# GEOS-ESM/QuickChem

Hardware: AMD Instinct MI355X
Metric: OH gridcells/sec (XGBoost predict), C360 L72 batch (higher is better)
Workload: dtype f32

## Files before the change

quickchem_amd/csrc/kernels.hip:

```cpp
#include <hip/hip_runtime.h>

#include <atomic>

#include <cstdint>

#include "kernels.hpp"

namespace ohx {

namespace {

constexpr int kWave = 64;
constexpr int kBlock = 256;
constexpr int kWavesPerBlock = kBlock / kWave;

typedef float f4u __attribute__((ext_vector_type(4), aligned(4)));
typedef unsigned int u32x2 __attribute__((ext_vector_type(2)));
typedef unsigned int u32x4 __attribute__((ext_vector_type(4)));
typedef const __attribute__((address_space(3))) char* lds_cptr;
typedef const __attribute__((address_space(3))) u32x4* lds_u32x4_ptr;
typedef __attribute__((address_space(3))) uint32_t* lds_u32_ptr;
typedef __attribute__((address_space(3))) void* lds_void_ptr;

__device__ __forceinline__ __amdgpu_buffer_rsrc_t make_rsrc(const void* p, uint32_t bytes) {
// ... 126 lines not shown
        x[g] = ((a.is2d_mask >> f) & 1u) ? src[at2] : __builtin_nontemporal_load(src + at3);
      }
    }
#pragma unroll
    for (uint32_t g = 0; g < GROUP; ++g) {
      const uint32_t f = f0 + g;
      float v = x[g];
      if (f == a.pl_feature) {
        asm volatile("");
        v = v / 100.0f;
      }
      any_inf |= f < nfeat && is_inf(v);
      if (!missing_is_nan && v == a.missing) v = qnan;
      if (!valid) v = 0.0f;
      lane_nan |= f < nfeat && (v != v);
      if (f < nfeat) tile[f * kWave] = v;
    }
  }
  if (any_inf && !is_inf(a.missing) && a.flags) atomicOr(a.flags, kFlagInfInput);
  return lane_nan;
}

struct CellAt {
  uint64_t at3, at2;
};
__device__ __forceinline__ CellAt cell_at(const FieldsArgs& a, uint64_t plane, uint64_t m) {
  const uint64_t k = m / plane, col = m - k * plane;
  return CellAt{a.level_stride ? k * a.level_stride + col : m, col};
}
__device__ __forceinline__ uint64_t level_floats(const FieldsArgs& a, uint64_t plane) {
  return a.level_stride ? a.level_stride : plane;
}

__device__ __forceinline__ float pow10_f32(float x) {
  double y = (double)x * 3.321928094887362;
  y = y < -1100.0 ? -1100.0 : (y > 1100.0 ? 1100.0 : y);
  const double n = __builtin_rint(y);
  const double f = y - n;
  double p = 4.44553827187081e-10;
  p = __builtin_fma(p, f, 7.054911620801121e-09);
  p = __builtin_fma(p, f, 1.0178086009239696e-07);
  p = __builtin_fma(p, f, 1.3215486790144305e-06);
  p = __builtin_fma(p, f, 1.5252733804059838e-05);
  p = __builtin_fma(p, f, 0.00015403530393381606);
  p = __builtin_fma(p, f, 0.0013333558146428441);
  p = __builtin_fma(p, f, 0.009618129107628477);
  p = __builtin_fma(p, f, 0.055504108664821576);
  p = __builtin_fma(p, f, 0.2402265069591007);
  p = __builtin_fma(p, f, 0.6931471805599453);
  p = __builtin_fma(p, f, 1.0);
  return (float)__builtin_ldexp(p, (int)n);
}

__device__ __forceinline__ void store_oh(const FieldsArgs& a, float* __restrict__ out, float* __restrict__ margin_out,
                                         uint64_t slab_out, uint64_t m, uint64_t at3, float acc) {
  if (margin_out) margin_out[m] = acc;
  float oh = acc;
  if (a.apply_pow10) oh = pow10_f32(acc);
  oh = oh * a.scale;
  out[slab_out + at3] = oh;
}

struct Row27 {
  f4u v[7];
};

__device__ __forceinline__ void load_row27(Row27& r, const float* __restrict__ rows, uint64_t row) {
  const float* p = rows + row * 27u;
#pragma unroll
  for (int q = 0; q < 6; ++q) r.v[q] = __builtin_nontemporal_load(reinterpret_cast<const f4u*>(p + 4 * q));
#pragma unroll
  for (int q = 0; q < 3; ++q) r.v[6][q] = __builtin_nontemporal_load(p + 24 + q);
}

__device__ __forceinline__ bool store_row27(float* __restrict__ tile, const Row27& r, bool valid, float missing,
                                            bool missing_is_nan, uint32_t* flags) {
  bool any_nan = false, any_inf = false;
  const float qnan = __builtin_nanf("");
#pragma unroll
  for (int f = 0; f < 27; ++f) {
    float x = r.v[f / 4][f % 4];
    if (!valid) x = 0.0f;
    any_inf |= is_inf(x);
    if (!missing_is_nan && x == missing) x = qnan;
    any_nan |= (x != x);
    tile[f * kWave] = x;
  }
  if (any_inf && !is_inf(missing) && flags) atomicOr(flags, kFlagInfInput);
  return any_nan;
}

// ... 25 lines not shown
  }
}

__device__ __forceinline__ bool store_pieces(float* __restrict__ tile_base, const Row27& r, const PredictArgs& a,
                                             uint64_t vmask, int lane, bool missing_is_nan) {
  bool any_nan = false, any_inf = false;
  const float qnan = __builtin_nanf("");
  asm volatile("" : "+v"(lane));
  const uint32_t ppr = 27u << (a.run_log - 2u);
  const bool all_valid = vmask == ~0ull;
#pragma unroll
  for (int q = 0; q < 7; ++q) {
    const uint32_t p = (uint32_t)lane + 64u * (uint32_t)q;
    if (p < kPiecesPerTile) {
      const uint32_t g = div27(p) >> (a.run_log - 2u);
      const uint32_t w4 = 4u * (p - g * ppr);
      const uint32_t col0 = run_first_lane(g, a.run_log, a.run_lo_bits);
      uint32_t rr = div27(w4);
      uint32_t f = w4 - 27u * rr;
#pragma unroll
      for (int c = 0; c < 4; ++c) {
        const uint32_t col = col0 | (rr << a.run_lo_bits);
        float x = r.v[q][c];
        if (!all_valid && !((vmask >> col) & 1ull)) x = 0.0f;
        any_inf |= is_inf(x);
        if (!missing_is_nan && x == a.missing) x = qnan;
        any_nan |= (x != x);
        tile_base[f * kWave + col] = x;
        ++f;
        if (f == 27u) {
          f = 0u;
          ++rr;
        }
      }
    }
  }
  if (any_inf && !is_inf(a.missing) && a.flags) atomicOr(a.flags, kFlagInfInput);
  return any_nan;
}


template <int CHAINS, bool HAS_MISSING>
__device__ __forceinline__ float walk_packed(__amdgpu_buffer_rsrc_t nodes, const uint32_t* __restrict__ roots,
                                             uint32_t t0, uint32_t t1, float acc, const float* __restrict__ tile) {
  for (uint32_t t = t0; t < t1; t += CHAINS) {
    uint2 nd[CHAINS];
    uint32_t cur[CHAINS];
#pragma unroll
    for (int c = 0; c < CHAINS; ++c) {
      const uint32_t tt = (t + c < t1) ? t + c : t1 - 1;
      cur[c] = roots[tt];
      nd[c] = load_node8(nodes, cur[c]);
    }
    bool more;
    do {
      float x[CHAINS];
#pragma unroll
      for (int c = 0; c < CHAINS; ++c) x[c] = tile[(nd[c].y & 31u) * kWave];
      more = false;
#pragma unroll
      for (int c = 0; c < CHAINS; ++c) {
        const uint32_t m = nd[c].y;
        bool go_left = x[c] < __uint_as_float(nd[c].x);
        if (HAS_MISSING) go_left = go_left || ((x[c] != x[c]) && (m & 32u));
        const uint32_t n = (m >> 6) - (go_left ? 1u : 0u);
        cur[c] = (m != 0u) ? n : cur[c];
// ... 24 lines not shown
  }
  return acc;
}


__device__ __forceinline__ bool go_left_or_default(float x, float thr, bool default_left) {
  const bool lt = x < thr;
  const bool missing = x != x;
  return lt | (missing & default_left);
}

using lane_mask = uint64_t;
constexpr int kFcmpOrdered = 7, kFcmpNotLess = 11 , kIcmpEq = 32;

__device__ __forceinline__ uint32_t pick(lane_mask m, uint32_t if_clear, uint32_t if_set) {
  uint32_t r;
  asm("v_cndmask_b32_e64 %0, %1, %2, %3" : "=v"(r) : "v"(if_clear), "v"(if_set), "s"(m));
  return r;
}

__device__ __forceinline__ lane_mask right_or_default(float x, float thr, uint32_t w, uint32_t default_left_bit) {
  const lane_mask not_less = __builtin_amdgcn_fcmpf(x, thr, kFcmpNotLess);
  const lane_mask number = __builtin_amdgcn_fcmpf(x, x, kFcmpOrdered);
  const lane_mask default_right = __builtin_amdgcn_uicmp(w & default_left_bit, 0u, kIcmpEq);
  return not_less & (number | default_right);
}

__device__ __forceinline__ uint32_t double_and_carry(uint32_t v, lane_mask carry) {
  uint32_t r;
  asm("v_addc_co_u32_e64 %0, vcc, %1, %1, %2" : "=v"(r) : "v"(v), "s"(carry) : "vcc");
  return r;
}

template <int CHAINS, bool HAS_MISSING, bool LAST>
__device__ __forceinline__ void super_step(u32x4 (&s)[CHAINS], uint32_t (&rel)[CHAINS], uint32_t (&leafb)[CHAINS],
                                           const char* __restrict__ tile_b) {
  float x0[CHAINS], x1[CHAINS];
  uint32_t thr1[CHAINS], f1[CHAINS];
  bool l0[CHAINS];
  lane_mask r0[CHAINS];
#pragma unroll
  for (int c = 0; c < CHAINS; ++c) {
    asm volatile("" : "+v"(s[c]));
    x0[c] = *reinterpret_cast<const float*>(tile_b + (s[c].w & 0x1F00u));
  }
#pragma unroll
  for (int c = 0; c < CHAINS; ++c) {
    const uint32_t w = s[c].w;
    if constexpr (HAS_MISSING) {
      r0[c] = right_or_default(x0[c], __uint_as_float(s[c].x), w, 32u);
      thr1[c] = pick(r0[c], s[c].y, s[c].z);
      f1[c] = (w >> pick(r0[c], 0u, 13u)) & 31u;
    } else {
      const bool l = x0[c] < __uint_as_float(s[c].x);
      l0[c] = l;
      thr1[c] = l ? s[c].y : s[c].z;
      f1[c] = (w >> (l ? 0u : 13u)) & 31u;
    }
    if (!LAST) x1[c] = *reinterpret_cast<const float*>(tile_b + (f1[c] << 8));
  }
#pragma unroll
  for (int c = 0; c < CHAINS; ++c) {
    const uint32_t w = s[c].w;
    leafb[c] = (f1[c] == 31u) ? thr1[c] : leafb[c];
    if (!LAST) {
      const uint32_t g = w >> 18;
      if constexpr (HAS_MISSING) {
        const lane_mask r1 = right_or_default(x1[c], __uint_as_float(thr1[c]), w, pick(r0[c], 64u, 128u));
        rel[c] = double_and_carry(double_and_carry(g, r0[c]), r1);
      } else {
        const bool l1 = x1[c] < __uint_as_float(thr1[c]);
        const lane_mask right0 = __builtin_amdgcn_ballot_w64(!l0[c]), right1 = __builtin_amdgcn_ballot_w64(!l1);
        rel[c] = double_and_carry(double_and_carry(g, right0), right1);
      }
    }
  }
}

template <int CHAINS, bool HAS_MISSING, class Fetch>
__device__ __forceinline__ void super_step_by_chain(u32x4 (&s)[CHAINS], uint32_t (&rel)[CHAINS], uint32_t (&leafb)[CHAINS],
                                                    const char* __restrict__ tile_b, Fetch fetch) {
  asm volatile("" : "+v"(s[0]));
  float x0_next = *reinterpret_cast<const float*>(tile_b + (s[0].w & 0x1F00u));
#pragma unroll
  for (int c = 0; c < CHAINS; ++c) {
    const uint32_t w = s[c].w;
    const float x0 = x0_next;
    if (c + 1 < CHAINS) {
      asm volatile("" : "+v"(s[c + 1]));
      x0_next = *reinterpret_cast<const float*>(tile_b + (s[c + 1].w & 0x1F00u));
    }
    uint32_t thr1, f1;
    bool l0 = false;
    lane_mask r0 = 0;
    if constexpr (HAS_MISSING) {
      r0 = right_or_default(x0, __uint_as_float(s[c].x), w, 32u);
      thr1 = pick(r0, s[c].y, s[c].z);
      f1 = (w >> pick(r0, 0u, 13u)) & 31u;
    } else {
      l0 = x0 < __uint_as_float(s[c].x);
      thr1 = l0 ? s[c].y : s[c].z;
      f1 = (w >> (l0 ? 0u : 13u)) & 31u;
    }
    const float x1 = *reinterpret_cast<const float*>(tile_b + (f1 << 8));
    const uint32_t g = w >> 18;
    if constexpr (HAS_MISSING) {
      const lane_mask r1 = right_or_default(x1, __uint_as_float(thr1), w, pick(r0, 64u, 128u));
      rel[c] = double_and_carry(double_and_carry(g, r0), r1);
    } else {
      const bool l1 = x1 < __uint_as_float(thr1);
      const lane_mask right0 = __builtin_amdgcn_ballot_w64(!l0), right1 = __builtin_amdgcn_ballot_w64(!l1);
      rel[c] = double_and_carry(double_and_carry(g, right0), right1);
    }
    s[c] = fetch(c, rel[c]);
    leafb[c] = (f1 == 31u) ? thr1 : leafb[c];
    __builtin_amdgcn_sched_barrier(0);
  }
}

constexpr uint32_t kFirstTrees = kFirstStepTrees;
constexpr uint32_t kFirstBytes = kFirstTrees * 2 * 16;

template <int CHAINS>
__device__ __forceinline__ void take_from_lanes(u32x4 (&s)[CHAINS], const u32x4 (&top)[CHAINS],
                                                const uint32_t (&rel)[CHAINS]) {
#pragma unroll
  for (int c = 0; c < CHAINS; ++c) {
    const int a = (int)(rel[c] << 2);
    s[c].x = (uint32_t)__builtin_amdgcn_ds_bpermute(a, (int)top[c].x);
    s[c].y = (uint32_t)__builtin_amdgcn_ds_bpermute(a, (int)top[c].y);
    s[c].z = (uint32_t)__builtin_amdgcn_ds_bpermute(a, (int)top[c].z);
    s[c].w = (uint32_t)__builtin_amdgcn_ds_bpermute(a, (int)top[c].w);
  }
}

template <int CHAINS, bool HAS_MISSING, bool TOPS>
__device__ __forceinline__ float walk_super(const uint4* __restrict__ nodes, const SuperTreeHead* __restrict__ heads,
                                            uint32_t t0, uint32_t t1, float acc, const float* __restrict__ tile,
                                            const char* __restrict__ first, uint32_t nfirst, uint32_t nodes_bytes,
                                            float* __restrict__ leaf_out = nullptr) {
  if (t0 >= t1) return acc;
  const __amdgpu_buffer_rsrc_t forest = make_rsrc(nodes, nodes_bytes);
  const uint32_t lane_id = threadIdx.x & (kWave - 1);
  const uint32_t top_off = (lane_id < kSuperTopSlots ? lane_id : kSuperTopSlots - 1u) << 4;
  const lds_cptr first_lds = (lds_cptr)first;
  const u32x4* __restrict__ nodes_v = reinterpret_cast<const u32x4*>(nodes);
  const char* tile_b = reinterpret_cast<const char*>(tile);
  SuperTreeHead hn[CHAINS];
// ... 329 lines not shown
  const uint64_t addr = reinterpret_cast<uint64_t>(fr.super);
  rg.desc.x = (uint32_t)__builtin_amdgcn_readfirstlane((int)(uint32_t)addr);
  rg.desc.y = (uint32_t)__builtin_amdgcn_readfirstlane((int)((uint32_t)(addr >> 32) & 0xFFFFu));
  rg.desc.z = (uint32_t)__builtin_amdgcn_readfirstlane((int)fr.super_bytes);
  rg.desc.w = 0x00020000u;
  rg.forest = make_rsrc(fr.super, fr.super_bytes);
  rg.heads = heads;
  rg.t0 = t0;
  rg.t1 = t1;
  rg.ngroups = (t1 - t0 + kRingChains - 1) / kRingChains;
  rg.total = rounds * rg.ngroups;
  rg.g = 0;
  rg.gave_up = false;
  if (threadIdx.x < kWave) {
    ring_stage(rg, t0, 0u, lane);
    asm volatile("s_waitcnt vmcnt(0)" ::: "memory");
  }
  if (threadIdx.x < (uint32_t)kRingWaves) ring_store(rg.progress + threadIdx.x, 0u);
  if (threadIdx.x == 0) {
    ring_store(rg.filled, 1u);
    ring_store(rg.claim, 1u);
    ring_store(rg.abort, 0u);
  }
  __syncthreads();
}

template <bool HAS_MISSING>
__device__ __forceinline__ float ring_walk_group(const SuperTreeHead (&h)[kRingChains], uint32_t ntrees_here,
                                                 __amdgpu_buffer_rsrc_t forest, const float* __restrict__ tile,
                                                 lds_cptr tops, float acc, lds_u32_ptr publish_to,
                                                 uint32_t publish_value, bool ahead) {
  constexpr int CHAINS = kRingChains;
  const char* tile_b = reinterpret_cast<const char*>(tile);
  __builtin_amdgcn_s_setprio(1);
  u32x4 s[CHAINS];
  uint32_t rel[CHAINS], leafb[CHAINS];
  float xr[CHAINS];
#pragma unroll
  for (int c = 0; c < CHAINS; ++c) xr[c] = tile[(h[c].root_meta & 31u) * kWave];
#pragma unroll
  for (int c = 0; c < CHAINS; ++c) {
    bool l = xr[c] < h[c].root_thr;
    if (HAS_MISSING) l = go_left_or_default(xr[c], h[c].root_thr, (h[c].root_meta & 32u) != 0u);
    rel[c] = 4u + (((h[c].root_meta & 0x100u) && !l) ? 1u : 0u);
    leafb[c] = 0u;
  }
  uint32_t nsteps = h[0].steps;
#pragma unroll
  for (int c = 1; c < CHAINS; ++c) nsteps = h[c].steps > nsteps ? h[c].steps : nsteps;
  nsteps = nsteps < kRingSteps ? kRingSteps : nsteps;
#pragma unroll
  for (int c = 0; c < CHAINS; ++c) s[c] = *(lds_u32x4_ptr)(tops + (uint32_t)c * kRingTreeBytes + (rel[c] << 4));
#pragma unroll
  for (uint32_t step = 1; step < kRingSteps; ++step) {
    if (step == 2 && !ahead) __builtin_amdgcn_s_setprio(2);
    super_step<CHAINS, HAS_MISSING, false>(s, rel, leafb, tile_b);
#pragma unroll
    for (int c = 0; c < CHAINS; ++c) s[c] = *(lds_u32x4_ptr)(tops + (uint32_t)c * kRingTreeBytes + (rel[c] << 4));
  }
  if (publish_to != nullptr) {
    asm volatile("s_waitcnt vmcnt(0)" ::: "memory");
    if ((threadIdx.x & (kWave - 1)) == 0) ring_store(publish_to, publish_value);
  }
  if (ahead) __builtin_amdgcn_s_setprio(2);
  else __builtin_amdgcn_s_setprio(3);
  uint32_t base[CHAINS];
#pragma unroll
  for (int c = 0; c < CHAINS; ++c) base[c] = h[c].base;
  for (uint32_t step = kRingSteps; step < nsteps; ++step)
    super_step_by_chain<CHAINS, HAS_MISSING>(s, rel, leafb, tile_b, [&](int c, uint32_t record) -> u32x4 {
      return __builtin_amdgcn_raw_buffer_load_b128(forest, (int)((base[c] + record) << 4), 0, 0);
    });
  super_step<CHAINS, HAS_MISSING, true>(s, rel, leafb, tile_b);
  __builtin_amdgcn_s_setprio(1);
#pragma unroll
  for (int c = 0; c < CHAINS; ++c)
    if ((uint32_t)c < ntrees_here) acc += __uint_as_float(leafb[c]);
  return acc;
}

__device__ __forceinline__ bool ring_aborted(const TopRing& rg) {
  return __builtin_amdgcn_readfirstlane((int)ring_load(rg.abort)) != 0;
}

__device__ __forceinline__ void ring_give_up(TopRing& rg, int lane) {
  rg.gave_up = true;
  if (lane == 0) ring_store(rg.abort, 1u);
}

__device__ __forceinline__ float ring_walk_tile(TopRing& rg, float acc, const float* __restrict__ tile, bool live,
                                                bool wave_nan, int lane, int wave) {
  if (rg.gave_up) return acc;
  for (uint32_t p = 0; p < rg.ngroups; ++p, ++rg.g) {
    const uint32_t g = rg.g;
    const uint32_t t = rg.t0 + p * kRingChains;
    uint32_t won = 0;
    uint32_t filled_now = 0;
    if (lane == 0) {
      uint32_t expected = g + 1u;
      const bool may = g + 1u < rg.total && !rg.gave_up;
      filled_now = ring_load(rg.filled);
      if (may) won = __hip_atomic_compare_exchange_strong(rg.claim, &expected, g + 2u, __ATOMIC_RELAXED, __ATOMIC_RELAXED,
                                                          __HIP_MEMORY_SCOPE_WORKGROUP) ? 1u : 0u;
    }
    won = (uint32_t)__builtin_amdgcn_readfirstlane((int)won);
    filled_now = (uint32_t)__builtin_amdgcn_readfirstlane((int)filled_now);
// ... 107 lines not shown
        keep = this_valid && !mine;
        wave_nan = false;
      }
    }
    const float acc = ring_walk_tile(rg, fr.base_score, tile, live, wave_nan, lane, wave);
    if (live && keep && !rg.gave_up) __builtin_nontemporal_store(acc, out + this_row);
    tile_id = next;
  }
  if (rg.gave_up && a.flags && lane == 0) atomicExch(a.flags + 2, a.train_id);
}

__global__ __launch_bounds__(kRingBlock) __attribute__((amdgpu_waves_per_eu(4))) void predict_fields_ring_kernel(
    DeviceForest fr, FieldsArgs a, const SuperTreeHead* __restrict__ heads, float* __restrict__ out,
    float* __restrict__ margin_out) {
  extern __shared__ float lds[];
  const int lane = threadIdx.x & (kWave - 1);
  const int wave = threadIdx.x / kWave;
  float* tile = lds + (size_t)wave * 27 * kWave + lane;
  const bool missing_is_nan = a.missing != a.missing;
  const uint64_t plane = (uint64_t)a.im * (uint64_t)a.jm;
  const uint64_t nrow = plane * (uint64_t)(a.k2 - a.k1 + 1);
  const uint64_t slab = level_floats(a, plane) * (uint64_t)(a.k1 - a.src_k0);
  const uint64_t slab_out = level_floats(a, plane) * (uint64_t)(a.k1 - a.out_k0);
  uint32_t block = blockIdx.x;
  if (a.xcd_remap && (gridDim.x & 7u) == 0u) block = (blockIdx.x & 7u) * (gridDim.x >> 3) + (blockIdx.x >> 3);
  const uint64_t wave_id = (uint64_t)block * kRingWaves + wave;
  const uint64_t nwaves = (uint64_t)gridDim.x * kRingWaves;
  const uint64_t first_tile = a.tile_begin + (uint64_t)block * kRingWaves;
  if (first_tile >= a.tile_end) return;
  const uint32_t rounds = (uint32_t)((a.tile_end - first_tile + nwaves - 1) / nwaves);
  TopRing rg;
  ring_begin(rg, reinterpret_cast<char*>(lds + (size_t)kRingWaves * 27 * kWave), fr, heads, a.tree_begin, a.tree_end, rounds);
  uint64_t tile_id = a.tile_begin + wave_id;
  for (uint32_t r = 0; r < rounds; ++r, tile_id += nwaves) {
    bool valid = false;
    uint64_t m = 0;
    if (tile_id < a.tile_end) m = tile_row(a.shape, tile_id, lane, nrow, &valid);
    const bool live = __any(valid);
    const CellAt at = cell_at(a, plane, valid ? m : 0);
    const bool lane_nan = live && fill_tile_fields(a, tile, 27u, at.at3, at.at2, slab, valid, missing_is_nan);
    bool wave_nan = __any(lane_nan);
    bool keep = valid;
    if (wave_nan && a.defer_count != nullptr && a.defer_cap == 0u) {
      if ((tile_id & 7u) == 0u) {
        const uint32_t n = 8u * (uint32_t)__popcll(__ballot(lane_nan && valid));
        if (lane == 0) atomicAdd(a.defer_count, n);
      }
    } else if (wave_nan && a.defer_count != nullptr) {
      const bool leaves = lane_nan && valid;
      const uint64_t who = __ballot(leaves);
      const uint32_t n = (uint32_t)__popcll(who);
      uint32_t at = 0;
      if (lane == 0) at = atomicAdd(a.defer_count, n);
      at = (uint32_t)__builtin_amdgcn_readfirstlane((int)at);
      if (at + n <= a.defer_cap) {
        if (leaves) a.defer_list[at + (uint32_t)__popcll(who & ((1ull << lane) - 1ull))] = (uint32_t)m;
        keep = valid && !lane_nan;
        wave_nan = false;
      }
    }
    const float acc = ring_walk_tile(rg, fr.base_score, tile, live, wave_nan, lane, wave);
    if (keep && !rg.gave_up) store_oh(a, out, margin_out, slab_out, m, at.at3, acc);
  }
  if (rg.gave_up && a.flags && lane == 0) atomicExch(a.flags + 2, a.train_id);
}

__global__ __launch_bounds__(kBlock) void combine_leaves_kernel(PredictArgs a, float base_score, float* __restrict__ out) {
  const int lane = threadIdx.x & (kWave - 1);
  const uint64_t ntiles = a.tile_end - a.tile_begin, nwaves = (uint64_t)gridDim.x * kWavesPerBlock;
  const uint32_t ntree = a.tree_end - a.tree_begin;
  for (uint64_t w = (uint64_t)blockIdx.x * kWavesPerBlock + threadIdx.x / kWave; w < ntiles; w += nwaves) {
    bool valid;
    const uint64_t row = launch_row(a, a.tile_begin + w, lane, &valid);
    if (!__any(valid)) continue;
    const float* leaves = a.leaf_buf + (size_t)w * ntree * kWave + lane;
    float acc = base_score;
#pragma unroll 4
    for (uint32_t t = 0; t < ntree; ++t) acc += leaves[(size_t)t * kWave];
    if (valid) out[row] = acc;
  }
}

template <bool PRED_LEAF>
__global__ __launch_bounds__(kBlock) void predict_rows_direct_kernel(DeviceForest fr, PredictArgs a) {
  const uint4* nodes = reinterpret_cast<const uint4*>(fr.wide);
  const bool missing_is_nan = a.missing != a.missing;
  const bool missing_is_inf = is_inf(a.missing);
  const uint32_t ntree = a.tree_end - a.tree_begin;
  const uint64_t stride = (uint64_t)gridDim.x * blockDim.x;
  for (uint64_t row = (uint64_t)blockIdx.x * blockDim.x + threadIdx.x; row < a.nrow; row += stride) {
    const float* x = a.rows + row * (uint64_t)a.ncol;
    float acc = fr.base_score;
    bool any_inf = false;
    for (uint32_t t = a.tree_begin; t < a.tree_end; ++t) {
      uint4 nd = nodes[fr.roots[t]];
// ... 1166 lines not shown
```

quickchem_amd/csrc/capi.cpp:

```cpp
#include <hip/hip_runtime_api.h>

#include <algorithm>
#include <cmath>
#include <cstdio>
#include <cstdlib>
#include <cstring>
#include <fstream>
#include <memory>
#include <atomic>
#include <chrono>
#include <mutex>
#include <unordered_map>
#include <sstream>
#include <string>
#include <unordered_set>
#include <vector>

#include "../../include/ohxgb.h"
#include "categorical.hpp"
#include "contribs.hpp"
#include "flatten.hpp"
#include "forest.hpp"
#include "groups.hpp"
#include "kernels.hpp"
// ... 1795 lines not shown
    b->tune.lds_pad = atoi(value);
  } else if (n == "ohx_register_host") {
    g_host_registry.on.store(atoi(value) != 0);
    if (atoi(value) == 0) g_host_registry.release_all();
  } else if (n == "ohx_reserve_cus") {
    const int k = atoi(value);
    if (k < 0 || k > 128) throw OhxError("ohx_reserve_cus must be 0..128");
    b->tune.reserve_cus = k;
  } else if (n == "ohx_ring_rounds") {
    const int k = atoi(value);
    if (k < 0) throw OhxError("ohx_ring_rounds must be >= 0");
    b->tune.ring_rounds = k;
  } else if (n == "ohx_copy_blocks") {
    g_copy_blocks.store((uint32_t)std::max(0, atoi(value)));
  } else if (n == "ohx_run1_pieces") {
    const int k = atoi(value);
    if (k < 0 || k > 64) throw OhxError("ohx_run1_pieces must be 0 .. 64 (0 and 1: one piece)");
    b->tune.run1_pieces = k;
  } else if (n == "ohx_tree_split") {
    if (v == "auto") b->tune.tree_split = -1;
    else if (v == "off") b->tune.tree_split = 0;
    else {
      const int k = atoi(value);
      if (k < 2 || k > 10) throw OhxError("ohx_tree_split must be auto, off or 2..10");
      b->tune.tree_split = k;
    }
  } else if (n == "ohx_defer_missing") {
    if (v != "auto" && v != "on" && v != "off") throw OhxError("ohx_defer_missing must be auto, on or off");
    b->tune.defer_missing = v == "auto" ? -1 : (v == "on" ? 1 : 0);
  } else if (n == "ohx_prefetch") {
    b->tune.prefetch = atoi(value) != 0;
  } else if (n == "ohx_coop_rows") {
    b->tune.coop_rows = atoi(value) != 0;
  } else if (n == "ohx_xcd_remap") {
    b->tune.xcd_remap = atoi(value) != 0;
  } else if (n == "ohx_overlap_group") {
    const int k = atoi(value);
    if (k < 0) throw OhxError("ohx_overlap_group must be >= 0");
    b->tune.overlap_group = k;
    if (b->uploaded) {
      HIP_CHECK(hipSetDevice(b->dev.ordinal));
      ensure_train_stream(*b);
    }
  } else if (n == "ohx_tree_tops") {
    const std::string v = value;
    if (v != "auto" && v != "on" && v != "off") throw OhxError("ohx_tree_tops must be auto, on or off");
    b->tune.tree_tops = v == "auto" ? -1 : (v == "on" ? 1 : 0);
  } else if (n == "ohx_contribs_split") {
    const std::string v = value;
    if (v != "auto" && v != "off") throw OhxError("ohx_contribs_split must be auto or off");
    b->contribs_split = v == "auto";
  } else if (n == "ohx_cat_kernel") {
    if (v != "auto" && v != "direct") throw OhxError("ohx_cat_kernel must be auto or direct");
    b->cat_force_direct = v == "direct";
  } else if (n == "ohx_device") {
    int k = atoi(value);
    if (k != b->device_pref) invalidate_device_state(*b);
    b->device_pref = k;
  }
  API_END();
}

int XGBoosterPredict(BoosterHandle handle, DMatrixHandle dmat, int option_mask, unsigned ntree_limit, int training,
                     bst_ulong* out_len, const float** out_result) {
  API_BEGIN();
  (void)training;
// ... 132 lines not shown
  a.km = km;
  a.k1 = k1 - 1;
  a.k2 = k2 - 1;
  a.missing = missing;
  tree_range(b, 0, &a.tree_begin, &a.tree_end);
  a.apply_pow10 = apply_pow10;
  a.scale = ohscale;
  a.flags = b.d_flags.p;
}

int OHXBoosterPredictFieldsDevice(BoosterHandle handle, const float* const d_fields[], const int32_t is2d[],
                                  int nfield, int pl_feature, int im, int jm, int km, int k1, int k2, float missing,
                                  int apply_pow10, float ohscale, float* d_oh_ml, float* d_margin, void* stream) {
  API_BEGIN();
  BoosterObj* b = as_booster(handle);
  refuse_groups(*b, "OHXBoosterPredictFieldsDevice");
  refuse_categorical(*b, "OHXBoosterPredictFieldsDevice");
  if (d_fields == nullptr || is2d == nullptr || d_oh_ml == nullptr) throw OhxError("predict_fields: NULL argument");
  ensure_uploaded(*b);
  FieldsArgs a{};
  fields_common(*b, a, is2d, nfield, pl_feature, im, jm, km, k1, k2, missing, apply_pow10, ohscale);
  for (int f = 0; f < nfield; ++f) {
    if (d_fields[f] == nullptr) throw OhxError("predict_fields: field " + std::to_string(f) + " is NULL");
    a.field[f] = d_fields[f];
  }
  a.out = d_oh_ml;
  a.margin_out = d_margin;
  if (pick_kernel(*b) == KernelKind::Wide) ensure_wide(*b);
  if (a.k2 >= a.k1) {
    const uint64_t nrow = (uint64_t)im * (uint64_t)jm * (uint64_t)(a.k2 - a.k1 + 1);
    LaunchTuning tune = b->tune;
    leaf_room(*b, nrow, a.tree_end - a.tree_begin, tune, im, jm, 0);
    const bool deferring = nfield == 27 && defer_prepare(*b, nrow, tune, static_cast<hipStream_t>(stream));
    HIP_CHECK(launch_predict_fields(pick_kernel(*b), device_forest(*b), a, b->dev.num_cus,
                                    static_cast<hipStream_t>(stream), tune));
    if (deferring) defer_look(*b, nrow, static_cast<hipStream_t>(stream));
  }
  API_END();
}

int OHXBoosterPredictFields(BoosterHandle handle, const float* const fields[], const int32_t is2d[], int nfield,
                            int pl_feature, int im, int jm, int km, int k1, int k2, float missing, int apply_pow10,
                            float ohscale, float* oh_ml, float* margin) {
  API_BEGIN();
  BoosterObj* b = as_booster(handle);
  refuse_groups(*b, "OHXBoosterPredictFields");
  refuse_categorical(*b, "OHXBoosterPredictFields");
  if (fields == nullptr || is2d == nullptr || oh_ml == nullptr) throw OhxError("predict_fields: NULL argument");
  ensure_uploaded(*b);
  FieldsArgs a{};
  fields_common(*b, a, is2d, nfield, pl_feature, im, jm, km, k1, k2, missing, apply_pow10, ohscale);
  if (a.k2 < a.k1) return 0;
  const size_t plane = (size_t)im * (size_t)jm;
  const size_t nlev = (size_t)(a.k2 - a.k1 + 1);
  const size_t nrow = plane * nlev;
  if (b->d_stage.size() < (size_t)nfield) b->d_stage.resize((size_t)nfield);
  const size_t min_rows = (size_t)64 * 256 * 20 * 2;
  size_t lev_per_piece = (min_rows + plane - 1) / plane;
  if (lev_per_piece * 8 < nlev) lev_per_piece = (nlev + 7) / 8;
  if (lev_per_piece < 1) lev_per_piece = 1;
  const bool registered = g_host_registry.on.load(std::memory_order_relaxed);
  const bool one_launch = registered && lev_per_piece >= nlev && nfield <= (int)kCopyListMax &&
                          ((size_t)nfield * nrow + nrow * 2) * sizeof(float) <= HostMover::kKernelBytesMax;
  HostMover in(b->s_exec, true);
  for (int f = 0; f < nfield; ++f) {
    if (fields[f] == nullptr) throw OhxError("predict_fields: field " + std::to_string(f) + " is NULL");
// ... 13 lines not shown
  a.out_k0 = a.k1;
  b->d_stage_out.ensure(nrow);
  a.out = b->d_stage_out.p;
  if (margin) {
    b->d_stage_margin.ensure(nrow);
    a.margin_out = b->d_stage_margin.p;
  }
  if (pick_kernel(*b) == KernelKind::Wide) ensure_wide(*b);
  const float* margin_base = a.margin_out;
  std::vector<hipEvent_t> events;
  for (size_t l0 = 0; l0 < nlev; l0 += lev_per_piece) {
    const size_t l1 = std::min(nlev, l0 + lev_per_piece);
    for (int f = 0; f < nfield; ++f) {
      if (is2d[f] || one_launch) continue;
      const float* src = fields[f] + plane * ((size_t)a.k1 + l0);
      HIP_CHECK(hipMemcpyAsync(b->d_stage[(size_t)f].p + plane * l0, src, plane * (l1 - l0) * sizeof(float),
                               hipMemcpyHostToDevice, b->s_copy));
    }
    if (!one_launch) {
      hipEvent_t ev;
      HIP_CHECK(hipEventCreateWithFlags(&ev, hipEventDisableTiming));
      events.push_back(ev);
      HIP_CHECK(hipEventRecord(ev, b->s_copy));
      HIP_CHECK(hipStreamWaitEvent(b->s_exec, ev, 0));
    }
    FieldsArgs piece = a;
    piece.k1 = a.k1 + (int)l0;
    piece.k2 = a.k1 + (int)l1 - 1;
    piece.margin_out = margin_base ? const_cast<float*>(margin_base) + plane * l0 : nullptr;
    LaunchTuning tune = b->tune;
    const uint64_t piece_rows = plane * (l1 - l0);
    leaf_room(*b, piece_rows, piece.tree_end - piece.tree_begin, tune, im, jm, 0);
    const bool deferring = nfield == 27 && defer_prepare(*b, piece_rows, tune, b->s_exec);
    HIP_CHECK(launch_predict_fields(pick_kernel(*b), device_forest(*b), piece, b->dev.num_cus, b->s_exec, tune));
    if (deferring) defer_look(*b, piece_rows, b->s_exec);
  }
  if (one_launch) {
    HostMover back(b->s_exec, false);
    back.add_slice(b->d_stage_out.p, oh_ml, plane * (size_t)km, plane * (size_t)a.k1, nrow);
    if (margin) back.add(margin, b->d_stage_margin.p, nrow);
    back.go();
  } else {
    if (registered) {
      (void)g_host_registry.want(oh_ml, plane * (size_t)km * sizeof(float));
      if (margin) (void)g_host_registry.want(margin, nrow * sizeof(float));
    }
    HIP_CHECK(hipMemcpyAsync(oh_ml + plane * (size_t)a.k1, b->d_stage_out.p, nrow * sizeof(float), hipMemcpyDeviceToHost,
                             b->s_exec));
    if (margin)
      HIP_CHECK(hipMemcpyAsync(margin, b->d_stage_margin.p, nrow * sizeof(float), hipMemcpyDeviceToHost, b->s_exec));
  }
  HIP_CHECK(hipStreamSynchronize(b->s_exec));
  for (hipEvent_t ev : events) (void)hipEventDestroy(ev);
  raise_flag_errors(*b, b->s_exec);
  API_END();
}

static void contribs_fields_call(BoosterObj& b, const float* const fields[], const int32_t is2d[], int nfield,
                                 int pl_feature, int im, int jm, int km, int k1, int k2, float missing, int approximate,
                                 unsigned ntree_limit, float* const out[], bool host_form, hipStream_t stream) {
  if (fields == nullptr || is2d == nullptr || out == nullptr) throw OhxError("predict_fields: NULL argument");
  if (approximate != 0 && approximate != 1) throw OhxError("approximate must be 0 (exact TreeSHAP) or 1");
  if (!b.loaded) throw OhxError("the booster holds no model: call XGBoosterLoadModel first");
  if (!host_form && stream_capturing(stream))
    refuse_in_capture("compute feature contributions",
                      "OHXBoosterPredictContribsFieldsDevice is not capturable; call it outside the capture");
// ... 279 lines not shown
    HIP_CHECK(hipEventRecord(b.run1_join, side));
    HIP_CHECK(hipStreamWaitEvent(stream, b.run1_join, 0));
  }
  for (int q = 0; q < npieces; ++q) {
    const int jq = j_lo[(size_t)q + 1] - j_lo[(size_t)q];
    const uint64_t first = (uint64_t)j_lo[(size_t)q] * (uint64_t)r.im;
    if (q >= 1) HIP_CHECK(hipStreamWaitEvent(stream, b.run1_prep[(size_t)q], 0));
    if (k2 >= k1 && jq > 0) {
      FieldsArgs fa{};
      fa.is2d_mask = 0;
      for (int f = 0; f < 27; ++f) {
        fa.field[f] = fields[f] + first;
        if (is2d[f]) fa.is2d_mask |= (1u << f);
      }
      fa.pl_feature = 1;
      fa.nfield = 27;
      fa.im = r.im; fa.jm = jq; fa.km = r.km;
      fa.level_stride = npieces > 1 ? plane : 0;
      fa.k1 = k1 - 1; fa.k2 = k2 - 1;
      fa.missing = r.missing;
      tree_range(b, 0, &fa.tree_begin, &fa.tree_end);
      fa.apply_pow10 = 1;
      fa.scale = r.ohscale;
      fa.out = oh_ml + first;
      fa.flags = b.d_flags.p;
      const uint64_t slab_rows = (uint64_t)r.im * (uint64_t)jq * (uint64_t)(k2 - k1 + 1);
      LaunchTuning tune = b.tune;
      leaf_room(b, slab_rows, fa.tree_end - fa.tree_begin, tune, r.im, jq, 0);
      const bool deferring = defer_prepare(b, slab_rows, tune, stream);
      if (gated && q == 0) {
        HIP_CHECK(hipEventSynchronize(walk_inputs));
        TICK_MARK("walk-inputs-there");
      }
      HIP_CHECK(launch_predict_fields(kind, device_forest(b), fa, b.dev.num_cus, stream, tune));
      if (deferring && q + 1 == npieces) defer_look(b, slab_rows, stream);
    }
    TICK_MARK("walk-enqueued");
    if (feed != nullptr && post_inputs == nullptr) post_inputs = feed->post_inputs();
    if (npieces == 1) {
      if (post_inputs != nullptr) HIP_CHECK(hipStreamWaitEvent(stream, post_inputs, 0));
      post_piece(0, stream);
      break;
    }
    HIP_CHECK(hipEventRecord(b.run1_walk[(size_t)q], stream));
    HIP_CHECK(hipStreamWaitEvent(side, b.run1_walk[(size_t)q], 0));
    if (post_inputs != nullptr) HIP_CHECK(hipStreamWaitEvent(side, post_inputs, 0));
    post_piece(q, side);
    if (q + 2 < npieces) {
      prep_piece(q + 2, side);
      HIP_CHECK(hipEventRecord(b.run1_prep[(size_t)q + 2], side));
    }
  }
  if (npieces > 1 && side != stream) {
    HIP_CHECK(hipEventRecord(b.run1_join, side));
    HIP_CHECK(hipStreamWaitEvent(stream, b.run1_join, 0));
  }
}

int OHXBoosterRun1Device(BoosterHandle handle, const OHXRun1Args* args, void* stream) {
  API_BEGIN();
  BoosterObj* b = as_booster(handle);
  refuse_groups(*b, "OHXBoosterRun1Device");
  refuse_categorical(*b, "OHXBoosterRun1Device");
  if (args == nullptr) throw OhxError("OHXBoosterRun1Device: args is NULL");
  if (!objective_is_identity(b->forest.objective))
    throw OhxError("objective '" + b->forest.objective + "' is not supported by OHXBoosterRun1");
// ... 501 lines not shown
```

quickchem_amd/csrc/kernels.hpp:

```cpp
#pragma once
#include <hip/hip_runtime_api.h>

#include <cstdint>
#include <string>

#include "flatten.hpp"

namespace ohx {

enum : uint32_t {
  kFlagInfInput = 1u,
};

constexpr uint32_t kFirstStepTrees = 128;

struct DeviceForest {
  const PackedNode* packed = nullptr;
  const WideNode* wide = nullptr;
  const uint32_t* roots = nullptr;
  const int32_t* packed_orig_id = nullptr;
  const SuperNode* super = nullptr;
  const SuperTreeHead* super_heads = nullptr;
  uint32_t num_trees = 0;
  uint32_t num_feature = 0;
// ... 68 lines not shown
  uint32_t* flags = nullptr;
  uint32_t train_id = 0, only_if_train = 0;
  uint64_t tile_begin = 0;
  uint64_t tile_end = 0;
  int xcd_remap = 1;
  const uint32_t* perm = nullptr;
  const uint32_t* perm_count = nullptr;
  uint32_t perm_slots = 0;
  uint32_t* defer_list = nullptr;
  uint32_t* defer_count = nullptr;
  uint32_t defer_cap = 0;
  float* leaf_buf = nullptr;
  uint32_t tree_split = 1;
  uint32_t run_log = 0, run_lo_bits = 0;
  TileShape shape;
};

struct TrainStreams {
  hipStream_t side = nullptr;
  hipEvent_t fork = nullptr, join = nullptr;
};

constexpr int kRingRoundsNoGrid = 16;
constexpr int kRingRoundsPermuted = 4;

struct LaunchTuning {
  int launches_per_residency = 2;
  int xcd_remap = 1;
  int overlap_group = 0;
  const TrainStreams* train = nullptr;
  int tree_tops = -1;
  int prefetch = 1;
  int coop_rows = 1;
  int lds_pad = 0;
  int ring_rounds = 64;
  int run1_pieces = 0;
  int reserve_cus = 0;
  int tree_split = -1;
  float* leaf_buf = nullptr;
  size_t leaf_words = 0;
  int defer_missing = -1;
  int defer_count_only = 0;
  uint32_t* defer_buf = nullptr;
  size_t defer_words = 0;
  int cluster = -1;
  int cluster_trees = 2, cluster_steps = 7, cluster_zorder = 0;
  int grid_im = 0, grid_jm = 0;
  uint64_t grid_row0 = 0;
  int brick_li = -1, brick_lj = -1, brick_lk = -1;
  int brick_k_fastest = 1;
};

struct FieldsArgs {
  const float* field[32];
  uint32_t is2d_mask = 0;
  uint32_t pl_feature = 1;
  uint32_t nfield = 0;
  int im = 0, jm = 0, km = 0, k1 = 0, k2 = 0;
  uint64_t level_stride = 0;
  int src_k0 = 0;
  int out_k0 = 0;
  float missing = 0.0f;
  uint32_t tree_begin = 0, tree_end = 0;
  int apply_pow10 = 1;
  float scale = 1.0f;
  float* out = nullptr;
  float* margin_out = nullptr;
  uint32_t* flags = nullptr;
  uint32_t train_id = 0, only_if_train = 0;
  uint64_t tile_begin = 0, tile_end = 0;
  int xcd_remap = 1;
  TileShape shape;
  uint32_t* defer_list = nullptr;
  uint32_t* defer_count = nullptr;
  uint32_t defer_cap = 0;
  const uint32_t* perm = nullptr;
  const uint32_t* perm_count = nullptr;
  uint32_t perm_slots = 0;
  float* leaf_buf = nullptr;
  uint32_t tree_split = 1;
};

struct PrepArgs {
  int im = 0, jm = 0, km = 0;
  uint64_t col0 = 0, ncols = 0;
  int beside_a_walk = 0;
  const float *ple_bst = nullptr, *zle_bst = nullptr, *tauclw = nullptr, *taucli = nullptr;
  const float* sca[7] = {};
  const float *gmito3 = nullptr, *gmitto3 = nullptr;
  float *pl_bst = nullptr, *tauclwdn = nullptr, *tauclidn = nullptr, *taucliup = nullptr, *tauclwup = nullptr;
  float *aodup = nullptr, *aoddn = nullptr, *strato3 = nullptr;
};

struct SlabArgs {
  int im = 0, jm = 0, km = 0;
  int dynamic_k_range = 1;
  float tropp_min = 4000.0f;
  const float *ple_mod = nullptr, *tropp = nullptr;
  int32_t* result = nullptr;
};

struct PostArgs {
  int im = 0, jm = 0, km = 0;
  uint64_t col0 = 0, ncols = 0;
  float avogad = 0, runiv = 0, epsilon = 0;
  const float *ple_mod = nullptr, *t_mod = nullptr, *q_mod = nullptr, *tropp = nullptr;
  const float *default_oh = nullptr, *oh_ml = nullptr;
  float *oh = nullptr, *ndwet = nullptr;
};

struct SolarArgs {
  int im = 0, jm = 0, jday = 0;
  float deg2rad = 0, rad2deg = 0;
  const float *lats = nullptr, *lons = nullptr;
// ... 54 lines not shown
```

Baseline: 2.418 billion.

## Freeze finished lanes and skip their node fetches in ring tree walk

Tree traversal now tracks a per-chain lane mask of lanes that have reached a leaf. Instead of carrying leaf values forward every step, finished lanes keep their last record, and node fetches (LDS and global buffer loads) run with EXEC masked to unfinished lanes. The leaf value is read once at the final step. This aims to cut memory traffic for lanes that finish early, at the cost of inline-asm EXEC manipulation, extra sched barriers, and an explicit lgkmcnt wait that may limit instruction overlap.

Result: no change. 2.403 billion (-0.6%).

```diff
diff --git a/quickchem_amd/csrc/kernels.hip b/quickchem_amd/csrc/kernels.hip
--- a/quickchem_amd/csrc/kernels.hip
+++ b/quickchem_amd/csrc/kernels.hip
@@ -388,9 +388,9 @@
   return r;
 }
 
-template <int CHAINS, bool HAS_MISSING, bool LAST>
+template <int CHAINS, bool HAS_MISSING, bool LAST, bool STAY = false>
 __device__ __forceinline__ void super_step(u32x4 (&s)[CHAINS], uint32_t (&rel)[CHAINS], uint32_t (&leafb)[CHAINS],
-                                           const char* __restrict__ tile_b) {
+                                           const char* __restrict__ tile_b, lane_mask* done = nullptr) {
   float x0[CHAINS], x1[CHAINS];
   uint32_t thr1[CHAINS], f1[CHAINS];
   bool l0[CHAINS];
@@ -418,7 +418,9 @@
 #pragma unroll
   for (int c = 0; c < CHAINS; ++c) {
     const uint32_t w = s[c].w;
-    leafb[c] = (f1[c] == 31u) ? thr1[c] : leafb[c];
+    if constexpr (!STAY) leafb[c] = (f1[c] == 31u) ? thr1[c] : leafb[c];
+    else if constexpr (LAST) leafb[c] = (f1[c] == 31u) ? thr1[c] : 0u;
+    else done[c] |= __builtin_amdgcn_uicmp(f1[c], 31u, kIcmpEq);
     if (!LAST) {
       const uint32_t g = w >> 18;
       if constexpr (HAS_MISSING) {
@@ -433,9 +435,34 @@
   }
 }
 
-template <int CHAINS, bool HAS_MISSING, class Fetch>
-__device__ __forceinline__ void super_step_by_chain(u32x4 (&s)[CHAINS], uint32_t (&rel)[CHAINS], uint32_t (&leafb)[CHAINS],
-                                                    const char* __restrict__ tile_b, Fetch fetch) {
+__device__ __forceinline__ void fetch_unfinished(u32x4& into, lane_mask done, __amdgpu_buffer_rsrc_t forest, uint32_t at) {
+  lane_mask all;
+  __builtin_amdgcn_sched_barrier(0);
+  asm volatile("s_andn1_saveexec_b64 %0, %1 ; finished lanes keep %2" : "=s"(all) : "s"(done), "v"(into), "v"(at) : "memory", "scc");
+  __builtin_amdgcn_sched_barrier(0);
+  into = __builtin_amdgcn_raw_buffer_load_b128(forest, (int)at, 0, 0);
+  __builtin_amdgcn_sched_barrier(0);
+  asm volatile("s_mov_b64 exec, %0 ; all lanes again" : : "s"(all) : "memory");
+  __builtin_amdgcn_sched_barrier(0);
+}
+
+template <uint32_t OFFSET>
+__device__ __forceinline__ void fetch_unfinished_lds(u32x4& into, lane_mask done, uint32_t at) {
+  static_assert(OFFSET < 65536u, "ds offset field");
+  lane_mask all;
+  asm volatile("s_andn1_saveexec_b64 %1, %2\n\tds_read_b128 %0, %3 offset:%4\n\ts_mov_b64 exec, %1"
+               : "+v"(into), "=&s"(all) : "s"(done), "v"(at), "n"(OFFSET) : "memory", "scc");
+}
+template <int CHAINS>
+__device__ __forceinline__ void ring_records_landed(u32x4 (&s)[CHAINS]) {
+  static_assert(CHAINS == 4, "one operand per chain");
+  asm volatile("s_waitcnt lgkmcnt(0)" : "+v"(s[0]), "+v"(s[1]), "+v"(s[2]), "+v"(s[3]));
+}
+
+template <int CHAINS, bool HAS_MISSING, class Offset>
+__device__ __forceinline__ void super_step_by_chain(u32x4 (&s)[CHAINS], uint32_t (&rel)[CHAINS], lane_mask (&done)[CHAINS],
+                                                    const char* __restrict__ tile_b, __amdgpu_buffer_rsrc_t forest,
+                                                    Offset offset) {
   asm volatile("" : "+v"(s[0]));
   float x0_next = *reinterpret_cast<const float*>(tile_b + (s[0].w & 0x1F00u));
 #pragma unroll
@@ -468,8 +495,8 @@
       const lane_mask right0 = __builtin_amdgcn_ballot_w64(!l0), right1 = __builtin_amdgcn_ballot_w64(!l1);
       rel[c] = double_and_carry(double_and_carry(g, right0), right1);
     }
-    s[c] = fetch(c, rel[c]);
-    leafb[c] = (f1 == 31u) ? thr1 : leafb[c];
+    done[c] |= __builtin_amdgcn_uicmp(f1, 31u, kIcmpEq);
+    fetch_unfinished(s[c], done[c], forest, offset(c, rel[c]));
     __builtin_amdgcn_sched_barrier(0);
   }
 }
@@ -865,9 +892,11 @@
                                                  uint32_t publish_value, bool ahead) {
   constexpr int CHAINS = kRingChains;
   const char* tile_b = reinterpret_cast<const char*>(tile);
+  const uint32_t tops_addr = (uint32_t)(uintptr_t)tops;
   __builtin_amdgcn_s_setprio(1);
   u32x4 s[CHAINS];
   uint32_t rel[CHAINS], leafb[CHAINS];
+  lane_mask done[CHAINS];
   float xr[CHAINS];
 #pragma unroll
   for (int c = 0; c < CHAINS; ++c) xr[c] = tile[(h[c].root_meta & 31u) * kWave];
@@ -876,7 +905,7 @@
     bool l = xr[c] < h[c].root_thr;
     if (HAS_MISSING) l = go_left_or_default(xr[c], h[c].root_thr, (h[c].root_meta & 32u) != 0u);
     rel[c] = 4u + (((h[c].root_meta & 0x100u) && !l) ? 1u : 0u);
-    leafb[c] = 0u;
+    done[c] = 0;
   }
   uint32_t nsteps = h[0].steps;
 #pragma unroll
@@ -887,9 +916,13 @@
 #pragma unroll
   for (uint32_t step = 1; step < kRingSteps; ++step) {
     if (step == 2 && !ahead) __builtin_amdgcn_s_setprio(2);
-    super_step<CHAINS, HAS_MISSING, false>(s, rel, leafb, tile_b);
-#pragma unroll
-    for (int c = 0; c < CHAINS; ++c) s[c] = *(lds_u32x4_ptr)(tops + (uint32_t)c * kRingTreeBytes + (rel[c] << 4));
+    super_step<CHAINS, HAS_MISSING, false, true>(s, rel, leafb, tile_b, done);
+    static_assert(CHAINS == 4, "one statement per chain");
+    fetch_unfinished_lds<0u * kRingTreeBytes>(s[0], done[0], tops_addr + (rel[0] << 4));
+    fetch_unfinished_lds<1u * kRingTreeBytes>(s[1], done[1], tops_addr + (rel[1] << 4));
+    fetch_unfinished_lds<2u * kRingTreeBytes>(s[2], done[2], tops_addr + (rel[2] << 4));
+    fetch_unfinished_lds<3u * kRingTreeBytes>(s[3], done[3], tops_addr + (rel[3] << 4));
+    ring_records_landed<CHAINS>(s);
   }
   if (publish_to != nullptr) {
     asm volatile("s_waitcnt vmcnt(0)" ::: "memory");
@@ -901,10 +934,10 @@
 #pragma unroll
   for (int c = 0; c < CHAINS; ++c) base[c] = h[c].base;
   for (uint32_t step = kRingSteps; step < nsteps; ++step)
-    super_step_by_chain<CHAINS, HAS_MISSING>(s, rel, leafb, tile_b, [&](int c, uint32_t record) -> u32x4 {
-      return __builtin_amdgcn_raw_buffer_load_b128(forest, (int)((base[c] + record) << 4), 0, 0);
+    super_step_by_chain<CHAINS, HAS_MISSING>(s, rel, done, tile_b, forest, [&](int c, uint32_t record) -> uint32_t {
+      return (base[c] + record) << 4;
     });
-  super_step<CHAINS, HAS_MISSING, true>(s, rel, leafb, tile_b);
+  super_step<CHAINS, HAS_MISSING, true, true>(s, rel, leafb, tile_b);
   __builtin_amdgcn_s_setprio(1);
 #pragma unroll
   for (int c = 0; c < CHAINS; ++c)
```

## Load brick field tiles as float4 pieces and prefetch next tile into registers

Applied to the files above, without the earlier changes.

Adds a 'fields together' path in the ring-walk fields kernel. When bricks are four cells wide along i and the field pointers are 16-byte aligned, each lane loads float4 pieces of several fields at once with nontemporal loads. The loads for the next tile are issued into registers before the current tile is walked, so global latency can overlap tree traversal. Row and cell indices are now recomputed at store time instead of being kept live across the walk, and the pow10 polynomial coefficients are read from constant memory, both apparently to lower register pressure. The cost is a 28-float register buffer per lane, extra NaN rescans of LDS, and more complex control flow.

After: 2.422 billion before, 2.420 billion after. No clear change (-0.1%).

```diff
diff --git a/quickchem_amd/csrc/capi.cpp b/quickchem_amd/csrc/capi.cpp
--- a/quickchem_amd/csrc/capi.cpp
+++ b/quickchem_amd/csrc/capi.cpp
@@ -1851,6 +1851,9 @@
     b->tune.prefetch = atoi(value) != 0;
   } else if (n == "ohx_coop_rows") {
     b->tune.coop_rows = atoi(value) != 0;
+  } else if (n == "ohx_fields_together") {
+    if (v != "auto" && v != "on" && v != "off") throw OhxError("ohx_fields_together must be auto, on or off");
+    b->tune.fields_together = v == "auto" ? -1 : (v == "on" ? 1 : 0);
   } else if (n == "ohx_xcd_remap") {
     b->tune.xcd_remap = atoi(value) != 0;
   } else if (n == "ohx_overlap_group") {
@@ -2049,6 +2052,7 @@
     LaunchTuning tune = b->tune;
     leaf_room(*b, nrow, a.tree_end - a.tree_begin, tune, im, jm, 0);
     const bool deferring = nfield == 27 && defer_prepare(*b, nrow, tune, static_cast<hipStream_t>(stream));
+    a.together = tune.fields_together != 0 && fields_pieces_aligned(a);
     HIP_CHECK(launch_predict_fields(pick_kernel(*b), device_forest(*b), a, b->dev.num_cus,
                                     static_cast<hipStream_t>(stream), tune));
     if (deferring) defer_look(*b, nrow, static_cast<hipStream_t>(stream));
@@ -2128,6 +2132,7 @@
     const uint64_t piece_rows = plane * (l1 - l0);
     leaf_room(*b, piece_rows, piece.tree_end - piece.tree_begin, tune, im, jm, 0);
     const bool deferring = nfield == 27 && defer_prepare(*b, piece_rows, tune, b->s_exec);
+    piece.together = tune.fields_together != 0 && fields_pieces_aligned(piece);
     HIP_CHECK(launch_predict_fields(pick_kernel(*b), device_forest(*b), piece, b->dev.num_cus, b->s_exec, tune));
     if (deferring) defer_look(*b, piece_rows, b->s_exec);
   }
@@ -2473,6 +2478,7 @@
         HIP_CHECK(hipEventSynchronize(walk_inputs));
         TICK_MARK("walk-inputs-there");
       }
+      fa.together = tune.fields_together != 0 && fields_pieces_aligned(fa);
       HIP_CHECK(launch_predict_fields(kind, device_forest(b), fa, b.dev.num_cus, stream, tune));
       if (deferring && q + 1 == npieces) defer_look(b, slab_rows, stream);
     }
diff --git a/quickchem_amd/csrc/kernels.hip b/quickchem_amd/csrc/kernels.hip
--- a/quickchem_amd/csrc/kernels.hip
+++ b/quickchem_amd/csrc/kernels.hip
@@ -182,31 +182,34 @@
   return a.level_stride ? a.level_stride : plane;
 }
 
+#define OHX_EXP2_POLY                                                                                              \
+  4.44553827187081e-10, 7.054911620801121e-09, 1.0178086009239696e-07, 1.3215486790144305e-06,                    \
+      1.5252733804059838e-05, 0.00015403530393381606, 0.0013333558146428441, 0.009618129107628477,                \
+      0.055504108664821576, 0.2402265069591007, 0.6931471805599453, 1.0
+__constant__ double kExp2PolyInMemory[12] = {OHX_EXP2_POLY};
+
+template <bool FROM_MEMORY = false>
 __device__ __forceinline__ float pow10_f32(float x) {
+  constexpr double literal[12] = {OHX_EXP2_POLY};
+  uint32_t none = 0;
+  if (FROM_MEMORY) asm volatile("" : "+s"(none));
+  const double* in_memory = kExp2PolyInMemory + none;
   double y = (double)x * 3.321928094887362;
   y = y < -1100.0 ? -1100.0 : (y > 1100.0 ? 1100.0 : y);
   const double n = __builtin_rint(y);
   const double f = y - n;
-  double p = 4.44553827187081e-10;
-  p = __builtin_fma(p, f, 7.054911620801121e-09);
-  p = __builtin_fma(p, f, 1.0178086009239696e-07);
-  p = __builtin_fma(p, f, 1.3215486790144305e-06);
-  p = __builtin_fma(p, f, 1.5252733804059838e-05);
-  p = __builtin_fma(p, f, 0.00015403530393381606);
-  p = __builtin_fma(p, f, 0.0013333558146428441);
-  p = __builtin_fma(p, f, 0.009618129107628477);
-  p = __builtin_fma(p, f, 0.055504108664821576);
-  p = __builtin_fma(p, f, 0.2402265069591007);
-  p = __builtin_fma(p, f, 0.6931471805599453);
-  p = __builtin_fma(p, f, 1.0);
+  double p = FROM_MEMORY ? in_memory[0] : literal[0];
+#pragma unroll
+  for (int k = 1; k < 12; ++k) p = __builtin_fma(p, f, FROM_MEMORY ? in_memory[k] : literal[k]);
   return (float)__builtin_ldexp(p, (int)n);
 }
 
+template <bool POLY_FROM_MEMORY = false>
 __device__ __forceinline__ void store_oh(const FieldsArgs& a, float* __restrict__ out, float* __restrict__ margin_out,
                                          uint64_t slab_out, uint64_t m, uint64_t at3, float acc) {
   if (margin_out) margin_out[m] = acc;
   float oh = acc;
-  if (a.apply_pow10) oh = pow10_f32(acc);
+  if (a.apply_pow10) oh = pow10_f32<POLY_FROM_MEMORY>(acc);
   oh = oh * a.scale;
   out[slab_out + at3] = oh;
 }
@@ -298,6 +301,85 @@
           f = 0u;
           ++rr;
         }
+      }
+    }
+  }
+  if (any_inf && !is_inf(a.missing) && a.flags) atomicOr(a.flags, kFlagInfInput);
+  return any_nan;
+}
+
+struct BrickAt {
+  uint32_t i0, j0, k0;
+};
+__device__ __forceinline__ BrickAt brick_at(const TileShape& sh, uint32_t tile) {
+  const uint32_t bi = tile % sh.nbi;
+  tile /= sh.nbi;
+  return BrickAt{bi << sh.li, (tile % sh.nbj) << sh.lj, (tile / sh.nbj) << sh.lk};
+}
+__device__ __forceinline__ bool fields_together(const FieldsArgs& a, uint32_t tile) {
+  return a.together != 0u && a.shape.im != 0u && a.shape.li == 2u && brick_at(a.shape, tile).i0 + 3u < a.shape.im;
+}
+
+__device__ __forceinline__ void load_field_pieces(Row27& r, const FieldsArgs& a, uint32_t tile, uint64_t slab, int lane) {
+  asm volatile("" : "+v"(lane));
+  const TileShape& sh = a.shape;
+  const BrickAt b = brick_at(sh, tile);
+  const uint32_t sub = (uint32_t)lane & 15u, g = (uint32_t)lane >> 4;
+  uint32_t j = b.j0 + (sub >> sh.lk), k = b.k0 + (sub & ((1u << sh.lk) - 1u));
+  j = j < sh.jm ? j : sh.jm - 1u;
+  k = k < sh.nk ? k : sh.nk - 1u;
+  const uint64_t plane = (uint64_t)sh.im * sh.jm;
+  const uint64_t at2 = (uint64_t)b.i0 + (uint64_t)sh.im * j;
+  const uint64_t at3 = slab + (uint64_t)k * (a.level_stride ? a.level_stride : plane) + at2;
+  uint32_t none = 0;
+  asm volatile("" : "+s"(none));
+  const float* first = a.field[none];
+#pragma unroll
+  for (int q = 0; q < 7; ++q) {
+    const float* of[4];
+#pragma unroll
+    for (uint32_t s = 0; s < 4u; ++s) of[s] = a.field[4u * (uint32_t)q + s + none];
+    const uint32_t f = 4u * (uint32_t)q + g;
+    const bool has = f < a.nfield;
+    const float* src = g == 0u ? of[0] : (g == 1u ? of[1] : (g == 2u ? of[2] : of[3]));
+    src = has ? src : first;
+    const bool flat = ((a.is2d_mask >> (has ? f : 0u)) & 1u) != 0u;
+    r.v[q] = __builtin_nontemporal_load(reinterpret_cast<const f4u*>(src + (flat ? at2 : at3)));
+  }
+}
+
+__device__ __forceinline__ bool store_field_pieces(float* __restrict__ tile_base, const Row27& r, const FieldsArgs& a,
+                                                   uint64_t vmask, int lane, bool missing_is_nan) {
+  const float qnan = __builtin_nanf("");
+  bool any_nan = false, any_inf = false;
+  asm volatile("" : "+v"(lane));
+  const TileShape& sh = a.shape;
+  const uint32_t sub = (uint32_t)lane & 15u, g = (uint32_t)lane >> 4;
+  const uint32_t dj = sub >> sh.lk, dk = sub & ((1u << sh.lk) - 1u);
+  const uint32_t col0 = sh.k_fastest ? dk | (dj << (sh.lk + 2u)) : (dj << 2) | (dk << (2u + sh.lj));
+  const uint32_t di_shift = sh.k_fastest ? sh.lk : 0u;
+  const bool all_valid = vmask == ~0ull;
+#pragma unroll
+  for (int q = 0; q < 7; ++q) {
+    const uint32_t f = 4u * (uint32_t)q + g;
+    if (f < 27u) {
+      f4u v = r.v[q];
+      if (f == a.pl_feature) {
+        asm volatile("");
+#pragma unroll
+        for (int c = 0; c < 4; ++c) v[c] = v[c] / 100.0f;
+      }
+#pragma unroll
+      for (int c = 0; c < 4; ++c) {
+        const uint32_t col = col0 | ((uint32_t)c << di_shift);
+        const bool valid = all_valid || ((vmask >> col) & 1ull);
+        float x = v[c];
+        if (f >= a.nfield) x = qnan;
+        any_inf |= valid && is_inf(x);
+        if (!missing_is_nan && x == a.missing) x = qnan;
+        if (!valid) x = 0.0f;
+        any_nan |= (x != x);
+        tile_base[f * kWave + col] = x;
       }
     }
   }
@@ -1078,35 +1160,76 @@
   TopRing rg;
   ring_begin(rg, reinterpret_cast<char*>(lds + (size_t)kRingWaves * 27 * kWave), fr, heads, a.tree_begin, a.tree_end, rounds);
   uint64_t tile_id = a.tile_begin + wave_id;
-  for (uint32_t r = 0; r < rounds; ++r, tile_id += nwaves) {
-    bool valid = false;
-    uint64_t m = 0;
-    if (tile_id < a.tile_end) m = tile_row(a.shape, tile_id, lane, nrow, &valid);
-    const bool live = __any(valid);
-    const CellAt at = cell_at(a, plane, valid ? m : 0);
-    const bool lane_nan = live && fill_tile_fields(a, tile, 27u, at.at3, at.at2, slab, valid, missing_is_nan);
+  Row27 regs;
+  bool valid = false, together = false;
+  if (tile_id < a.tile_end) {
+    (void)tile_row(a.shape, tile_id, lane, nrow, &valid);
+    together = __any(valid) && fields_together(a, (uint32_t)tile_id);
+    if (together) load_field_pieces(regs, a, (uint32_t)tile_id, slab, lane);
+  }
+  for (uint32_t r = 0; r < rounds; ++r) {
+    int l = lane;
+    asm volatile("" : "+v"(l));
+    const bool live = tile_id < a.tile_end && __any(valid);
+    const bool this_valid = valid, this_together = together;
+    bool lane_nan = false;
+    if (live && together) {
+      lane_nan = store_field_pieces(tile - lane, regs, a, __ballot(valid), l, missing_is_nan);
+    } else if (live) {
+      const uint64_t m = tile_row(a.shape, tile_id, l, nrow, &valid);
+      const CellAt at = cell_at(a, plane, valid ? m : 0);
+      lane_nan = fill_tile_fields(a, tile, 27u, at.at3, at.at2, slab, valid, missing_is_nan);
+    }
+    const uint64_t next = tile_id + nwaves;
+    valid = false;
+    together = false;
+    if (next < a.tile_end) {
+      (void)tile_row(a.shape, next, l, nrow, &valid);
+      together = __any(valid) && fields_together(a, (uint32_t)next);
+      if (together) load_field_pieces(regs, a, (uint32_t)next, slab, l);
+    }
     bool wave_nan = __any(lane_nan);
-    bool keep = valid;
+    __builtin_amdgcn_fence(__ATOMIC_RELEASE, "wavefront");
+    __builtin_amdgcn_wave_barrier();
+    __builtin_amdgcn_fence(__ATOMIC_ACQUIRE, "wavefront");
+    if (wave_nan && this_together && a.defer_count != nullptr) {
+      lane_nan = false;
+#pragma unroll
+      for (int f = 0; f < 27; ++f) {
+        const float x = tile[f * kWave];
+        lane_nan |= (x != x);
+      }
+    }
+    bool keep = this_valid;
     if (wave_nan && a.defer_count != nullptr && a.defer_cap == 0u) {
       if ((tile_id & 7u) == 0u) {
-        const uint32_t n = 8u * (uint32_t)__popcll(__ballot(lane_nan && valid));
-        if (lane == 0) atomicAdd(a.defer_count, n);
+        const uint32_t n = 8u * (uint32_t)__popcll(__ballot(lane_nan && this_valid));
+        if (l == 0) atomicAdd(a.defer_count, n);
       }
     } else if (wave_nan && a.defer_count != nullptr) {
-      const bool leaves = lane_nan && valid;
+      const bool leaves = lane_nan && this_valid;
       const uint64_t who = __ballot(leaves);
       const uint32_t n = (uint32_t)__popcll(who);
       uint32_t at = 0;
-      if (lane == 0) at = atomicAdd(a.defer_count, n);
+      if (l == 0) at = atomicAdd(a.defer_count, n);
       at = (uint32_t)__builtin_amdgcn_readfirstlane((int)at);
       if (at + n <= a.defer_cap) {
-        if (leaves) a.defer_list[at + (uint32_t)__popcll(who & ((1ull << lane) - 1ull))] = (uint32_t)m;
-        keep = valid && !lane_nan;
+        bool mine;
+        const uint64_t m = tile_row(a.shape, tile_id, l, nrow, &mine);
+        if (leaves) a.defer_list[at + (uint32_t)__popcll(who & ((1ull << l) - 1ull))] = (uint32_t)m;
+        keep = this_valid && !lane_nan;
         wave_nan = false;
       }
     }
     const float acc = ring_walk_tile(rg, fr.base_score, tile, live, wave_nan, lane, wave);
-    if (keep && !rg.gave_up) store_oh(a, out, margin_out, slab_out, m, at.at3, acc);
+    if (keep && !rg.gave_up) {
+      int lw = lane;
+      asm volatile("" : "+v"(lw));
+      bool mine;
+      const uint64_t m = tile_row(a.shape, tile_id, lw, nrow, &mine);
+      store_oh<true>(a, out, margin_out, slab_out, m, cell_at(a, plane, m).at3, acc);
+    }
+    tile_id = next;
   }
   if (rg.gave_up && a.flags && lane == 0) atomicExch(a.flags + 2, a.train_id);
 }
diff --git a/quickchem_amd/csrc/kernels.hpp b/quickchem_amd/csrc/kernels.hpp
--- a/quickchem_amd/csrc/kernels.hpp
+++ b/quickchem_amd/csrc/kernels.hpp
@@ -124,6 +124,7 @@
   int tree_tops = -1;
   int prefetch = 1;
   int coop_rows = 1;
+  int fields_together = -1;
   int lds_pad = 0;
   int ring_rounds = 64;
   int run1_pieces = 0;
@@ -171,7 +172,15 @@
   uint32_t perm_slots = 0;
   float* leaf_buf = nullptr;
   uint32_t tree_split = 1;
-};
+  uint32_t together = 0;
+};
+
+inline bool fields_pieces_aligned(const FieldsArgs& a) {
+  if (a.nfield == 0 || a.nfield > 32 || a.im <= 0 || a.im % 4 != 0 || a.level_stride % 4 != 0) return false;
+  for (uint32_t f = 0; f < a.nfield; ++f)
+    if (reinterpret_cast<uintptr_t>(a.field[f]) % 16 != 0) return false;
+  return true;
+}
 
 struct PrepArgs {
   int im = 0, jm = 0, km = 0;
```
